# arghyasur1991/Spark-TTS

Measured on AMD Instinct MI355X. Metric: audio samples/sec (whole node), Spark-TTS-0.5B greedy, higher is better.
Workload: dtype bf16 weights + KV, fp32 activations/accumulate (LLM); vocoder: fp32 operands split into 2 bf16 planes, 3 products on the bf16 matrix pipe, fp32 accumulate

## Files before the change

### include/sparkmi_debug.h

```cpp
#ifndef SPARKMI_DEBUG_H
#define SPARKMI_DEBUG_H

#include "sparkmi.h"

#ifdef __cplusplus
extern "C" {
#endif

int smi_llm_time_kernel(smi_llm* h, int kernel, int layer, int iters, float* ms_avg, void* stream);
int smi_llm_debug_stamps(smi_llm* h, int kernel, int layer, double* out);
int smi_llm_engine(smi_llm* h, int32_t* enabled, int32_t* info, char* why, int n);
int smi_llm_set_engine(smi_llm* h, int on);
int smi_llm_engine_plan(const smi_llm_cfg* cfg, int ncu, int32_t* stats);
int smi_llm_engine_stamps(smi_llm* h, double* out, int cap);
int smi_llm_debug_hidden(smi_llm* h, float* out_host, int n);
int smi_llm_debug_read(smi_llm* h, int what, void* out_host, size_t cap, size_t* got);

int smi_llm_debug_set_kv(smi_llm* h, int layer, int slot, int pos0, int n, const float* k_host, const float* v_host);
int smi_llm_debug_get_kv(smi_llm* h, int layer, int slot, int pos0, int n, float* k_host, float* v_host);
int smi_llm_debug_layer(smi_llm* h, int layer, int M, const int32_t* rows_host, const float* hidden_host, int stage);
int smi_llm_debug_raw_stamps(smi_llm* h, unsigned long long* out, int n);
int smi_llm_debug_sample(smi_llm* h, const float* logits_host, int n_rows, uint64_t seed, int use_bound, int32_t* tokens_out);
int smi_llm_debug_penalize(smi_llm* h, const float* logits_host, int n_rows, const uint16_t* hist_host, const smi_penalty_params* pens,
                           const int32_t* emitted_host, float* logits_out, int32_t* argmax_out);
int smi_llm_debug_logprob(smi_llm* h, const float* logits_host, int n_rows, const float* temperature_host, const int32_t* tokens_host,
                          float* lp_out);

#ifdef __cplusplus
}
#endif
#endif
```

### spark-tts_amd/csrc/smi_llm.hip

```cpp
#include "smi_common.h"
#include <stdio.h>
#include <string.h>
#include <cmath>
#include <map>
#include <mutex>
#include <vector>

namespace {

constexpr int kMaxRows = SMI_MAX_ROWS;
constexpr int kHeadDim = 64;

struct RowDesc {
  int32_t slot, pos, token, flags;
};

struct SampRec {
  int32_t mode;
  int32_t top_k;
  float inv_temp, top_p;
  unsigned long long seed;
  int32_t has_seed, pad;
};

// ... 1462 lines not shown
              pk.x = smi_f32_to_bf16(s.x) | (smi_f32_to_bf16(s.y) << 16);
              pk.y = smi_f32_to_bf16(s.z) | (smi_f32_to_bf16(s.w) << 16);
              *(uint2*)((uint16_t*)base + off) = pk;
            }
          }
        }
      }
    }
  }
}

__device__ __forceinline__ int lm_tile(const int* tlist, int idx) {
  const int c = tlist[0];
  idx = idx < c ? idx : c - 1;
  return tlist[1 + (idx > 0 ? idx : 0)];
}
__device__ __forceinline__ void lm_mask4(const Ctl* ctl, int slot, int n, float4& s) {
  const AllowRec* a = &ctl->allow[slot];
  if (!allow_has(a, n + 0)) s.x = -INFINITY;
  if (!allow_has(a, n + 1)) s.y = -INFINITY;
  if (!allow_has(a, n + 2)) s.z = -INFINITY;
  if (!allow_has(a, n + 3)) s.w = -INFINITY;
}
template <int HV, int RT = 0>
__global__ __launch_bounds__(256 * HV) void k_lm(GemmP p, int ngroups_arg, int m0_launch) {
  constexpr int NTB = 2, NW = 4, U = 8, MT = 1;
  constexpr size_t kHalfBytes = (size_t)NW * NTB * MT * 1024 + 32 * 4 + NTB * 32 * 8;
  extern __shared__ __attribute__((aligned(16))) unsigned char smem_all[];
  const int half = HV == 2 ? (int)threadIdx.x >> 8 : 0;
  unsigned char* smem = smem_all + half * kHalfBytes;
  const int tid = threadIdx.x & 255, lane = tid & 63, wave = tid >> 6;
  const int KT = p.KT, NT = p.NT;
  const int m0 = m0_launch + 16 * half;
  const int M = p.M - m0 < 16 ? (p.M - m0 > 0 ? p.M - m0 : 0) : 16;
  const int ntl = RT ? p.tlist[0] : 0;
  const int ngroups = RT ? (ntl + NTB - 1) / NTB : ngroups_arg;
  float4* red = (float4*)smem;
  float* rarr = (float*)(smem + (size_t)NW * NTB * MT * 1024);
  float* bestv = rarr + 32;
  int* besti = (int*)(bestv + NTB * 32);
  const int k8 = lane >> 4, em = lane & 15;
  const int mrow = em < M ? em : (M > 0 ? M - 1 : 0);
  const int xrow = m0 + mrow < p.M ? m0 + mrow : p.M - 1;
  bf16x8 bf[U][3];
#pragma unroll
  for (int u = 0; u < U; ++u) {
// ... 7 lines not shown
#pragma unroll
    for (int u = 0; u < U; ++u) {
      int j = wave + u * NW;
      j = j < KT ? j : KT - 1;
#pragma unroll
      for (int nb = 0; nb < NTB; ++nb) {
        int nt = g * NTB + nb;
        nt = RT ? lm_tile(p.tlist, nt) : (nt < NT ? nt : NT - 1);
        w[u][nb] = smi_ldw(&p.W[((size_t)nt * KT + j) * 64 + lane]);
      }
    }
  };
  int g = blockIdx.x;
  if (g < ngroups) load_w(g);
  for (int m = wave; m < M; m += NW) {
    float v = smi_ss_lane_sum(p.sspart + (size_t)(m0 + m) * p.npart, p.npart, lane);
    v = smi_wave_sum(v);
    if (lane == 0) rarr[m] = 1.0f / sqrtf(v / (float)(KT * 32) + p.eps);
  }
  for (int i = tid; i < NTB * 32; i += 256) { bestv[i] = -INFINITY; besti[i] = 0x7fffffff; }
  __syncthreads();
  const float rn = rarr[mrow];
  for (; g < ngroups; g += gridDim.x) {
    f32x4 acc[3][NTB];
#pragma unroll
    for (int c = 0; c < 3; ++c)
#pragma unroll
      for (int a = 0; a < NTB; ++a) acc[c][a] = (f32x4){0.f, 0.f, 0.f, 0.f};
#pragma unroll
    for (int u = 0; u < U; ++u) {
      if (wave + u * NW < KT) {
#pragma unroll
        for (int nb = 0; nb < NTB; ++nb) {
          const bf16x8 a = __builtin_bit_cast(bf16x8, w[u][nb]);
          acc[2][nb] = __builtin_amdgcn_mfma_f32_16x16x32_bf16(a, bf[u][2], acc[2][nb], 0, 0, 0);
          acc[1][nb] = __builtin_amdgcn_mfma_f32_16x16x32_bf16(a, bf[u][1], acc[1][nb], 0, 0, 0);
          acc[0][nb] = __builtin_amdgcn_mfma_f32_16x16x32_bf16(a, bf[u][0], acc[0][nb], 0, 0, 0);
        }
      }
    }
    const int gn = g + gridDim.x;
    if (gn < ngroups) load_w(gn);
#pragma unroll
    for (int nb = 0; nb < NTB; ++nb) {
      const f32x4 t = (acc[2][nb] + acc[1][nb]) + acc[0][nb];
      red[(wave * NTB + nb) * 64 + lane] = make_float4(t[0], t[1], t[2], t[3]);
    }
    __syncthreads();
    if (wave < NTB) {
      const int nb = wave, nt = RT ? (g * NTB + nb < ntl ? p.tlist[1 + g * NTB + nb] : NT) : g * NTB + nb;
      if (nt < NT) {
        float4 s = red[(0 * NTB + nb) * 64 + lane];
#pragma unroll
        for (int wv = 1; wv < NW; ++wv) {
          const float4 t = red[(wv * NTB + nb) * 64 + lane];
          s.x += t.x; s.y += t.y; s.z += t.z; s.w += t.w;
        }
        s.x *= rn; s.y *= rn; s.z *= rn; s.w *= rn;
        const int n = nt * 16 + 4 * (lane >> 4);
        const bool valid = em < M;
        if (RT && valid) lm_mask4(p.ctl, p.rows[m0 + em].slot, n, s);
        if (valid && p.Y) {
          float* y = p.Y + (size_t)(m0 + em) * p.V + n;
          if (n + 0 < p.V) y[0] = s.x;
          if (n + 1 < p.V) y[1] = s.y;
          if (n + 2 < p.V) y[2] = s.z;
          if (n + 3 < p.V) y[3] = s.w;
        }
        float bv = -INFINITY;
        int bi = 0x7fffffff;
        const float sv[4] = {s.x, s.y, s.z, s.w};
#pragma unroll
        for (int r = 0; r < 4; ++r)
          if (n + r < p.V && sv[r] > bv) { bv = sv[r]; bi = n + r; }
#pragma unroll
        for (int o = 16; o <= 32; o <<= 1) {
          const float ov = __shfl_xor(bv, o, 64);
          const int oi = __shfl_xor(bi, o, 64);
          if (ov > bv || (ov == bv && oi < bi)) { bv = ov; bi = oi; }
        }
        if (lane < 16 && valid) {
          const float cv = bestv[nb * 32 + em];
          const int ci = besti[nb * 32 + em];
          if (bv > cv || (bv == cv && bi < ci)) { bestv[nb * 32 + em] = bv; besti[nb * 32 + em] = bi; }
        }
      }
    }
    __syncthreads();
  }
  if (tid < M) {
    float bv = -INFINITY;
    int bi = 0x7fffffff;
#pragma unroll
    for (int nb = 0; nb < NTB; ++nb) {
      const float ov = bestv[nb * 32 + tid];
      const int oi = besti[nb * 32 + tid];
      if (ov > bv || (ov == bv && oi < bi)) { bv = ov; bi = oi; }
    }
    p.pval[(size_t)(m0 + tid) * gridDim.x + blockIdx.x] = bv;
    p.pidx[(size_t)(m0 + tid) * gridDim.x + blockIdx.x] = bi;
  }
}


template <int UW, int RT = 0>
__global__ __launch_bounds__(256) void k_lm32(GemmP p, int ngroups_arg, int m0) {
  constexpr int NTB = 2, NW = 4, U = UW;
  extern __shared__ __attribute__((aligned(16))) unsigned char smem[];
  const int tid = threadIdx.x, lane = tid & 63, wave = tid >> 6;
  const int KT = p.KT, NT = p.NT;
  const int ntl = RT ? p.tlist[0] : 0;
  const int ngroups = RT ? (ntl + NTB - 1) / NTB : ngroups_arg;
  const int M = p.M - m0 < 32 ? p.M - m0 : 32;
  float4* red = (float4*)smem;
  float* rarr = (float*)(smem + (size_t)NW * NTB * 2 * 1024);
  float* bestv = rarr + 32;
  int* besti = (int*)(bestv + NTB * 32);
  uint4* xl = (uint4*)(smem + (size_t)NW * NTB * 2 * 1024 + 32 * 4 + NTB * 32 * 8);
  const int k8 = lane >> 4, em = lane & 15;
  const int row0 = m0 + (em < M ? em : M - 1);
  constexpr int RPW = 8;
  float ssv[RPW][4];
  const bool ss_early = p.npart <= 256;
// ... 1522 lines not shown
  uint16_t* phist;
  int32_t* pen_idx; size_t pen_idx_cap;
  std::vector<int32_t> host_pen_idx;
  float* logits; int* tok;
  float* cand_v; int* cand_i; unsigned int* cand_n;
  unsigned long long* stamps; int stamps_on;
  int max_steps;
  int tune[4];
  int graph_steps;
  int pf_inline;
  int pf_qkv_eighths;
  int prefetch_mask, prefetch_rows;
  int tune2;
  int pgemm_min_rows;
  int pg_min[4];
  int wd_parts;
  int exact;
  int gu1_lo;
  int gu1_rows;
  hipGraphExec_t graph; int graph_B, graph_seg, graph_ident, graph_samp, graph_pen, graph_lp, graph_allow;
  std::map<hipGraphExec_t, hipStream_t> graph_last;
  std::map<uint64_t, hipGraphExec_t> graph_cache;
  hipEvent_t ev0, ev1;
  std::vector<RowDesc> host_rows;
#ifdef SMI_DIAG
  EngState eng;
  int eng_on;
#endif
};

namespace {

std::vector<const void*>& lds_big_kernels() {
  static std::vector<const void*> v;
  return v;
}
bool lds_big_register(const void* f) {
  lds_big_kernels().push_back(f);
  return true;
}
template <auto F>
struct LdsBig {
  static inline const bool reg = lds_big_register((const void*)F);
};
constexpr int kLdsBigBytes = 160 * 1024;

// ... 46 lines not shown
}
bool pen_any(const smi_llm* L) {
  for (int sl = 0; sl < kMaxRows; ++sl)
    if (L->slot_pen[sl]) return true;
  return false;
}
bool lp_any(const smi_llm* L) {
  for (int sl = 0; sl < kMaxRows; ++sl)
    if (L->slot_lp[sl]) return true;
  return false;
}
bool allow_any(const smi_llm* L) {
  for (int sl = 0; sl < kMaxRows; ++sl)
    if (L->slot_allow[sl]) return true;
  return false;
}
bool lm_restricted(const smi_llm* L) {
  return L->lm_restrict && L->KTh <= 32 && !L->exact && allow_any(L);
}
bool logits_needed(const smi_llm* L) {
  return samp_any(L) || pen_any(L) || lp_any(L) || (allow_any(L) && !lm_restricted(L));
}
int allow_bits(const smi_llm* L) { return allow_any(L) ? (lm_restricted(L) ? 3 : 1) : 0; }
uint64_t graph_key(const smi_llm* L, int samp, int pen, int lp, int K) {
  return (uint64_t)L->B | ((uint64_t)L->attn_seg << 8) | ((uint64_t)(L->identity_slots ? 1 : 0) << 24) | ((uint64_t)samp << 25) |
         ((uint64_t)pen << 26) | ((uint64_t)lp << 27) | ((uint64_t)allow_bits(L) << 28) | ((uint64_t)K << 32);
}
void graphs_flush(smi_llm* L) {
  std::vector<hipStream_t> drained;
  for (auto& gl : L->graph_last) {
    bool seen = false;
    for (hipStream_t d : drained) seen |= d == gl.second;
    if (!seen) { (void)hipStreamSynchronize(gl.second); drained.push_back(gl.second); }
  }
  L->graph_last.clear();
  for (auto& kv : L->graph_cache) if (kv.second) (void)hipGraphExecDestroy(kv.second);
  L->graph_cache.clear();
  L->graph = nullptr;
}

template <int MT, int NTB, int NW, int U, int WB, int PRO, int EPI, int H = 1, int OCC = 1>
int launch_gemm_kv(const smi_llm* L, GemmP p, hipStream_t st) {
  const int work = (p.NT + NTB - 1) / NTB * H;
  p.work_blocks = work;
  p.stamps = L->stamps_on ? L->stamps : nullptr;
  if constexpr (MT == 1 && NTB == 1 && NW == 16 && H == 4 && PRO == PRO_PLAIN && EPI == EPI_RESID) {
    if (p.M == 1 && !p.stamps && p.KT <= 160 && !(L->tune2 & 1048576)) {
      const int helpers = (L->prefetch_mask & 4) && p.pf.base && work < 232 ? ((L->tune2 & 4194304) ? 224 : (256 - work) / 8 * 8) : 0;
      if (p.KT <= 32) hipLaunchKernelGGL(k_down1<2>, dim3(work + helpers), dim3(256), 0, st, p);
// ... 458 lines not shown
      p.XSout = L->xs_h; p.ssout = L->sspart;
      p.gamma_next = layer + 1 < c.num_layers ? (const float*)sec(L, SMI_LLM_LN1, layer + 1)
                                              : (const float*)sec(L, SMI_LLM_FINAL_NORM, 0);
      if (layer + 1 < c.num_layers) p.pf = PfDesc{sec(L, SMI_LLM_WQKV, layer + 1), L->KTh * 1024, L->NTqkv, 0, (L->NTqkv + 7) / 8};
      if (M >= L->dc_min && M <= kMaxRows && !L->tune[3] && !L->stamps_on && p.KT <= 160 && p.NT % 4 == 0)
        return launch_down_chains(L, p, st);
      switch (L->tune[3]) {
        case 2: return launch_gemm<1, 16, 3, 4, PRO_PLAIN, EPI_RESID>(L, p, st);
        case 4: return launch_gemm<1, 8, 10, 2, PRO_PLAIN, EPI_RESID>(L, p, st);
        case 5: return launch_gemm<1, 16, 2, 5, PRO_PLAIN, EPI_RESID, 2>(L, p, st);
        case 6: return launch_gemm<1, 16, 2, 5, PRO_PLAIN, EPI_RESID>(L, p, st);
        default:
          if (M <= 8) return launch_gemm<1, 16, 2, 5, PRO_PLAIN, EPI_RESID, 4>(L, p, st);
          if (M <= 16) return launch_gemm<1, 16, 2, 5, PRO_PLAIN, EPI_RESID, 4, 0>(L, p, st);
          if (M <= 32) return launch_gemm<1, 16, 2, 5, PRO_PLAIN, EPI_RESID, 2, 0>(L, p, st);
          return launch_gemm<1, 16, 2, 5, PRO_PLAIN, EPI_RESID, 1, 0>(L, p, st);
      }
    case KLM:
      p.W = (const uint4*)sec(L, SMI_LLM_LM_HEAD, 0); p.NT = L->NTlm; p.KT = L->KTh;
      p.XS = L->xs_h;
      p.Y = logits ? logits : (logits_needed(L) ? L->logits : nullptr);
      p.V = c.vocab_size; p.pval = L->pval; p.pidx = L->pidx;
      p.stamps = L->stamps_on ? L->stamps : nullptr;
      if (L->KTh <= 32 && !logits && rows == L->rows && lm_restricted(L)) {
        p.tlist = L->tlist; p.ctl = L->ctl;
        const size_t lds = (size_t)4 * 2 * 1024 + 32 * 4 + 2 * 32 * 8;
        const size_t lds32 = (size_t)4 * 2 * 2 * 1024 + 32 * 4 + 2 * 32 * 8 + (size_t)L->KTh * 12 * 16 * 16;
        if (M <= 16) {
          hipLaunchKernelGGL((k_lm<1, 1>), dim3(L->lm_blocks), dim3(256), lds, st, p, 0, 0);
          SMI_LAUNCH_CHECK();
          return SMI_OK;
        }
        for (int m0 = 0; m0 < M; m0 += 32) {
          if (!(L->tune2 & 8192) && lds32 <= 150 * 1024) {
            if (L->KTh <= 28) hipLaunchKernelGGL((k_lm32<7, 1>), dim3(lm_blocks_for(L, M)), dim3(256), lds32, st, p, 0, m0);
            else hipLaunchKernelGGL((k_lm32<8, 1>), dim3(lm_blocks_for(L, M)), dim3(256), lds32, st, p, 0, m0);
          } else
            hipLaunchKernelGGL((k_lm<2, 1>), dim3(lm_blocks_for(L, M)), dim3(512), 2 * lds, st, p, 0, m0);
          SMI_LAUNCH_CHECK();
        }
        return SMI_OK;
      }
      if (L->KTh <= 32) {
        const int ngroups = (L->NTlm + 1) / 2;
        const size_t lds = (size_t)4 * 2 * 1024 + 32 * 4 + 2 * 32 * 8;
        if (M <= 16) {
// ... 408 lines not shown
  {
    static std::mutex mu;
    static bool done[64] = {};
    int dev = 0;
    std::lock_guard<std::mutex> lk(mu);
    if (hipGetDevice(&dev) != hipSuccess || dev < 0 || dev >= 64) {
      smi_set_error("smi_llm_create: no current device");
      smi_llm_destroy(L);
      return SMI_EHIP;
    }
    for (size_t i = 0; i < lds_big_kernels().size() && !done[dev]; ++i)
      if (hipFuncSetAttribute(lds_big_kernels()[i], hipFuncAttributeMaxDynamicSharedMemorySize, kLdsBigBytes) != hipSuccess) {
        smi_set_error("smi_llm_create: hipFuncSetAttribute(MaxDynamicSharedMemorySize) failed: %s", hipGetErrorString(hipGetLastError()));
        smi_llm_destroy(L);
        return SMI_EHIP;
      }
    done[dev] = true;
  }
  if (hipEventCreate(&L->ev0) != hipSuccess || hipEventCreate(&L->ev1) != hipSuccess) {
    smi_set_error("hipEventCreate failed");
    smi_llm_destroy(L);
    return SMI_EHIP;
  }
#ifdef SMI_DIAG
  L->eng_on = 0;
  snprintf(L->eng.why, sizeof(L->eng.why), "off (opt-in: SPARKMI_ENGINE=1 or smi_llm_set_engine)");
  { const char* e = smi_env("SPARKMI_ENGINE");
    if (e && e[0] == '1') {
      const int rce = eng_create(L);
      if (rce) { smi_llm_destroy(L); return rce; }
      L->eng_on = L->eng.enabled;
    }
  }
#endif
  *out = L;
  return SMI_OK;
}

int smi_llm_destroy(smi_llm* L) {
  if (!L) return SMI_OK;
  graphs_flush(L);
  eng_destroy(L);
  void* ptrs[] = {L->h, L->qbuf, L->xs_h, L->xs_attn, L->xs_act, L->sspart, L->part_o, L->h2, L->dpart, L->fuse_cnt, L->rows, L->plan, L->pf_tiles, L->pval, L->pidx, L->hist,
                  L->count, L->finished, L->step, L->ctl, L->ptab, L->kcache, L->vcache, L->logits, L->tok, L->cand_v, L->cand_i, L->cand_n, L->stamps, L->bh, L->bq, L->bxs_h, L->bxs_attn, L->bxs_act, L->bss, L->pslab, L->apart,
                  L->phist, L->pen_idx, L->lp, L->lp_part, L->lp_rowc, L->tlist};
  for (void* q : ptrs)
    if (q) (void)hipFree(q);
  if (L->ev0) (void)hipEventDestroy(L->ev0);
  if (L->ev1) (void)hipEventDestroy(L->ev1);
  delete L;
  return SMI_OK;
}

int smi_llm_set_sampling(smi_llm* L, int do_sample, float temperature, int top_k, float top_p, uint64_t seed) {
  SMI_REQUIRE(L, "smi_llm_set_sampling: null handle");
  if (do_sample) {
    SMI_REQUIRE(temperature > 0.f, "smi_llm_set_sampling: temperature must be > 0");
    SMI_REQUIRE(top_k >= 1 && top_k <= kSampleCap, "smi_llm_set_sampling: top_k must be in 1..%d", kSampleCap);
    SMI_REQUIRE(top_p > 0.f && top_p <= 1.f, "smi_llm_set_sampling: top_p must be in (0, 1]");
    if (top_k > L->cfg.vocab_size) top_k = L->cfg.vocab_size;
  }
  const bool changed = L->do_sample != (do_sample ? 1 : 0) ||
                       (do_sample && (L->temperature != temperature || L->top_k != top_k || L->top_p != top_p));
  L->do_sample = do_sample ? 1 : 0;
  L->temperature = temperature; L->top_k = top_k; L->top_p = top_p; L->seed = seed;
  L->hctl.seed = seed;
  SMI_HIP(hipMemcpy(&L->ctl->seed, &seed, sizeof(seed), hipMemcpyHostToDevice));
  if (changed) graphs_flush(L);
// ... 965 lines not shown

int smi_llm_engine(smi_llm* L, int32_t* enabled, int32_t* info, char* why, int n) {
  SMI_REQUIRE(L, "smi_llm_engine: null handle");
  if (enabled) *enabled = L->eng.enabled && L->eng_on;
  if (info) { info[0] = L->eng.ncu; info[1] = L->eng.maxlen; info[2] = L->eng.lds; info[3] = L->eng.enabled; }
  if (why && n > 0) { strncpy(why, L->eng.why, (size_t)n - 1); why[n - 1] = 0; }
  return SMI_OK;
}

int smi_llm_set_engine(smi_llm* L, int on) {
  SMI_REQUIRE(L, "smi_llm_set_engine: null handle");
  int v = on ? 1 : 0;
  if (v && !L->eng.enabled) {
    SMI_HIP(hipDeviceSynchronize());
    const int rce = eng_create(L);
    if (rce) return rce;
    v = L->eng.enabled;
  }
  if (v != L->eng_on) { SMI_HIP(hipDeviceSynchronize()); graphs_flush(L); }
  L->eng_on = v;
  return SMI_OK;
}

int smi_llm_engine_plan(const smi_llm_cfg* cfg, int ncu, int32_t* stats) {
  SMI_REQUIRE(cfg_ok(cfg) && stats, "smi_llm_engine_plan: invalid argument");
  EngPlanHost P;
  char why[128] = "";
  const int Q = cfg->num_heads * cfg->head_dim, KV = cfg->num_kv_heads * cfg->head_dim;
  if (!eng_build_plan(cfg->hidden_size, Q, KV, cfg->intermediate_size, cfg->num_heads, ncu, P, why, sizeof(why))) {
    smi_set_error("engine plan: %s", why);
    return SMI_EINVAL;
  }
  long total = 0, want = 0;
  for (int ph = 0; ph < 4; ++ph) want += (long)P.g.nparts[ph] * P.g.part_imgs[ph];
  std::vector<unsigned char> seen[4];
  for (int ph = 0; ph < 4; ++ph) seen[ph].assign((size_t)P.g.nparts[ph] * 4 * 64, 0);
  for (int c = 0; c < ncu; ++c)
    for (int w = 0; w < kEngWaves; ++w) {
      const EngWavePlan& wp = P.cu[c].w[w];
      for (int ph = 0; ph < 4; ++ph)
        for (int j = wp.jstart[ph]; j < wp.jstart[ph + 1]; ++j) {
          const EngJob& jb = wp.jobs[j];
          SMI_REQUIRE(P.cu[c].parts[P.cu[c].pstart[ph] + jb.slot] == jb.part, "engine plan: job slot does not name its part");
          SMI_REQUIRE((int)jb.goff + jb.nimg <= (int)P.cu[c].len_cu, "engine plan: job beyond the CU's stream");
          for (int r = 0; r < jb.nimg; ++r) {
            const uint32_t d = P.desc[(size_t)c * P.maxlen + jb.goff + r];
// ... 14 lines not shown

int smi_llm_debug_hidden(smi_llm* L, float* out_host, int n) {
  SMI_REQUIRE(L && out_host && n >= L->H, "smi_llm_debug_hidden: out holds %d floats, %d needed", n, L ? L->H : 0);
  SMI_HIP(hipDeviceSynchronize());
  SMI_HIP(hipMemcpy(out_host, L->h, (size_t)L->H * 4, hipMemcpyDeviceToHost));
  return eng_check(L);
}

int smi_llm_debug_read(smi_llm* L, int what, void* out_host, size_t cap, size_t* got) {
  SMI_REQUIRE(L && out_host && got, "smi_llm_debug_read: null argument");
  const void* src = nullptr;
  size_t n = 0;
  const size_t R = L->B > 0 ? (size_t)L->B : 1;
  switch (what) {
    case 0: src = L->qbuf; n = R * L->Q * 4; break;
    case 1: src = L->xs_attn; n = R * L->Q * 6; break;
    case 2: src = L->xs_act; n = R * L->I * 6; break;
    case 3: src = L->xs_h; n = R * L->H * 6; break;
    case 4: src = L->h; n = R * L->H * 4; break;
    case 5: src = L->eng.gran; n = L->eng.gran ? (size_t)2 * L->eng.gran_per_buf * 8 : 0; break;
    case 6: src = L->sspart; n = R * L->H; break;
    case 7: src = L->kcache; n = (size_t)L->cfg.max_positions * kHeadDim * 2; break;
    case 8: src = L->h2; n = (size_t)L->H * 4; break;
    default: smi_set_error("smi_llm_debug_read: what=%d", what); return SMI_EINVAL;
  }
  SMI_REQUIRE(src && n <= cap, "smi_llm_debug_read: buffer %d holds %zu bytes, out holds %zu", what, n, cap);
  SMI_HIP(hipDeviceSynchronize());
  SMI_HIP(hipMemcpy(out_host, src, n, hipMemcpyDeviceToHost));
  *got = n;
  return SMI_OK;
}

static int debug_kv_check(const smi_llm* L, int layer, int slot, int pos0, int n) {
  SMI_REQUIRE(L && !L->paged, "debug KV access needs a contiguous KV cache (kv_page_tokens = 0)");
  SMI_REQUIRE(layer >= 0 && layer < L->cfg.num_layers && slot >= 0 && slot < L->cfg.max_slots && pos0 >= 0 && n >= 0 &&
              pos0 + n <= L->cfg.max_positions, "debug KV access: layer %d slot %d positions %d..%d out of range", layer, slot, pos0, pos0 + n);
  return SMI_OK;
}

int smi_llm_debug_set_kv(smi_llm* L, int layer, int slot, int pos0, int n, const float* k_host, const float* v_host) {
  { const int rc = debug_kv_check(L, layer, slot, pos0, n); if (rc) return rc; }
  SMI_REQUIRE(k_host && v_host, "smi_llm_debug_set_kv: null argument");
  SMI_HIP(hipDeviceSynchronize());
  const int nkv = L->cfg.num_kv_heads, f32 = L->cfg.kv_dtype;
  const size_t esz = f32 ? 4 : 2;
  std::vector<unsigned char> buf((size_t)n * kHeadDim * esz);
// ... 256 lines not shown
```

### spark-tts_amd/sparkmi/_lib.py

```python
from __future__ import annotations

import ctypes as C
import os
from pathlib import Path

_HERE = Path(__file__).resolve().parent
LIB_PATH = Path(os.environ["SPARKMI_LIB"]) if os.environ.get("SPARKMI_LIB") else _HERE / "libsparkmi.so"

SMI_MAX_ROWS = 64
SMI_MAX_EOS = 4
ABI_VERSION = 4


class SparkMIError(RuntimeError):
    pass


class LLMCfg(C.Structure):
    _fields_ = [(n, C.c_int32) for n in (
        "vocab_size", "hidden_size", "num_layers", "num_heads", "num_kv_heads", "head_dim",
        "intermediate_size", "max_slots", "max_positions", "kv_dtype", "use_graph")] + [("rms_eps", C.c_float),
                                                                                        ("kv_page_tokens", C.c_int32), ("kv_pages", C.c_int32), ("wd_plain", C.c_int32),
                                                                                        ("weights_exact", C.c_int32)]

# ... 100 lines not shown
    "smi_voc_num_launches": (_I, [_VP]),
    "smi_voc_time_launch": (_I, [_VP, _I, _I, _P(C.c_float), _P(C.c_double), C.c_char_p, _I, _VP]),
    "smi_voc_block_arena_count": (_I, [_P(VocBlockCfg)]),
    "smi_voc_block_arena_bytes": (_SZ, [_P(VocBlockCfg)]),
    "smi_voc_block_arena_entry": (_I, [_P(VocBlockCfg), _I, C.c_char_p, _I, _P(_SZ), _P(_SZ), _P(C.c_int32)]),
    "smi_voc_block_run": (_I, [_P(VocBlockCfg), _VP, _SZ, _VP, _VP, _VP, _P(C.c_int32), _I, _I, _VP, _VP]),
    "smi_enc_arena_count": (_I, [_P(EncCfg)]),
    "smi_enc_arena_entry": (_I, [_P(EncCfg), _I, C.c_char_p, _I, _P(_SZ), _P(_SZ), _P(C.c_int32)]),
    "smi_enc_arena_bytes": (_SZ, [_P(EncCfg)]),
    "smi_enc_create": (_I, [_P(EncCfg), _VP, _SZ, _P(_VP)]),
    "smi_enc_destroy": (_I, [_VP]),
    "smi_enc_forward": (_I, [_VP, _VP, _I, _VP, _I, _VP, _VP, _P(_I), _VP]),
    "smi_enc_debug_stage": (_I, [_VP, C.c_char_p, _VP, _SZ, _P(C.c_int32), _VP]),
    "smi_enc_num_launches": (_I, [_VP]),
    "smi_enc_time_launch": (_I, [_VP, _I, _I, _P(C.c_float), _P(C.c_double), C.c_char_p, _I, _VP]),
}

DEBUG_SYMBOLS = {
    "smi_llm_time_kernel": (_I, [_VP, _I, _I, _I, _P(C.c_float), _VP]),
    "smi_llm_debug_stamps": (_I, [_VP, _I, _I, _P(C.c_double)]),
    "smi_llm_engine": (_I, [_VP, _P(C.c_int32), _P(C.c_int32), C.c_char_p, _I]),
    "smi_llm_set_engine": (_I, [_VP, _I]),
    "smi_llm_engine_plan": (_I, [_P(LLMCfg), _I, _P(C.c_int32)]),
    "smi_llm_engine_stamps": (_I, [_VP, _P(C.c_double), _I]),
    "smi_llm_debug_hidden": (_I, [_VP, _P(C.c_float), _I]),
    "smi_llm_debug_read": (_I, [_VP, _I, _VP, _SZ, _P(_SZ)]),
    "smi_llm_debug_raw_stamps": (_I, [_VP, _P(C.c_uint64), _I]),
    "smi_llm_debug_sample": (_I, [_VP, _P(C.c_float), _I, C.c_uint64, _I, _P(C.c_int32)]),
    "smi_llm_debug_logprob": (_I, [_VP, _P(C.c_float), _I, _P(C.c_float), _P(C.c_int32), _P(C.c_float)]),
    "smi_llm_debug_penalize": (_I, [_VP, _P(C.c_float), _I, _P(C.c_uint16), _P(PenaltyParams), _P(C.c_int32), _P(C.c_float),
                                    _P(C.c_int32)]),
    "smi_llm_debug_set_kv": (_I, [_VP, _I, _I, _I, _I, _P(C.c_float), _P(C.c_float)]),
    "smi_llm_debug_get_kv": (_I, [_VP, _I, _I, _I, _I, _P(C.c_float), _P(C.c_float)]),
    "smi_llm_debug_layer": (_I, [_VP, _I, _I, _P(C.c_int32), _P(C.c_float), _I]),
}

DIAG_PATH = LIB_PATH.with_name("libsparkmi_diag.so")


class _Lib:

    def __init__(self, cdll: C.CDLL, path: Path, is_diag: bool):
        self._cdll, self.path, self.is_diag = cdll, path, is_diag

    def __getattr__(self, name):
        return getattr(self._cdll, name)
# ... 56 lines not shown
```

### spark-tts_amd/sparkmi/llm.py

```python
from __future__ import annotations

import ctypes as C
import itertools
import json
import warnings
from pathlib import Path
from typing import Iterable, List, Mapping, Optional, Sequence, Union

import numpy as np
import torch

from . import _lib
from .arena import llm_cfg_struct, pack_llm_arena
from .config import LLMConfig


EosLike = Union[None, int, Iterable[int]]
SAMPLING_KEYS = ("do_sample", "temperature", "top_k", "top_p", "seed")
PENALTY_KEYS = ("repetition_penalty", "presence_penalty", "frequency_penalty", "min_new_tokens", "penalize_prompt")
PENALTY_NEUTRAL = dict(repetition_penalty=1.0, presence_penalty=0.0, frequency_penalty=0.0, min_new_tokens=0)
LOGPROB_KEYS = ("return_log_probs",)
ALLOW_KEY = "allowed_token_ids"


# ... 585 lines not shown
        self._lib.check(self._lib.smi_llm_forward_logits(
            self._h, a.ctypes.data_as(C.POINTER(C.c_int64)), a.shape[0], C.c_void_p(out.data_ptr()),
            self._stream()), "smi_llm_forward_logits")
        return out

    def _need_diag(self, what: str) -> None:
        if not self._lib.is_diag:
            raise _lib.SparkMIError(f"SparkLLM.{what} is a diagnostics entry (include/sparkmi_debug.h): construct the engine with "
                                    "diag=True (libsparkmi_diag.so); the product library does not export it")

    def engine_info(self) -> dict:
        self._need_diag("engine_info")
        on = C.c_int32(0)
        info = (C.c_int32 * 4)()
        why = C.create_string_buffer(200)
        self._lib.check(self._lib.smi_llm_engine(self._h, C.byref(on), info, why, 200), "smi_llm_engine")
        return {"enabled": bool(on.value), "built": bool(info[3]), "cus": int(info[0]), "images_per_wave": int(info[1]),
                "lds_bytes": int(info[2]), "why": why.value.decode(errors="replace")}

    def set_engine(self, on: bool) -> None:
        self._need_diag("set_engine")
        self._lib.check(self._lib.smi_llm_set_engine(self._h, 1 if on else 0), "smi_llm_set_engine")

    def engine_stamps(self) -> np.ndarray:
        self._need_diag("engine_stamps")
        n = 3 * self.cfg.num_hidden_layers * 16
        out = (C.c_double * n)()
        self._lib.check(self._lib.smi_llm_engine_stamps(self._h, out, n), "smi_llm_engine_stamps")
        return np.array(out, dtype=np.float64).reshape(3, self.cfg.num_hidden_layers, 16)

    def debug_hidden(self) -> np.ndarray:
        self._need_diag("debug_hidden")
        out = np.zeros(self.cfg.hidden_size, dtype=np.float32)
        self._lib.check(self._lib.smi_llm_debug_hidden(self._h, out.ctypes.data_as(C.POINTER(C.c_float)), out.size), "smi_llm_debug_hidden")
        return out

    def debug_read(self, what: int) -> np.ndarray:
        self._need_diag("debug_read")
        buf = np.zeros(1 << 22, dtype=np.uint8)
        got = C.c_size_t(0)
        self._lib.check(self._lib.smi_llm_debug_read(self._h, int(what), buf.ctypes.data_as(C.c_void_p), buf.size, C.byref(got)),
                   "smi_llm_debug_read")
        return buf[: got.value].copy()

    def debug_set_kv(self, layer: int, slot: int, k: np.ndarray, v: np.ndarray, pos0: int = 0) -> None:
        self._need_diag("debug_set_kv")
# ... 126 lines not shown
```

Before: 564,600.

## Screen lm_head argmax with int8 bounds and recompute only candidate tiles exactly

Adds an int8 copy of the lm_head with per-row scales and error bounds, built once at create. For single-row greedy decode it runs an int8 MFMA screen that computes interval bounds on each logit, finds the max lower bound, then recomputes the exact bf16 3-plane GEMM only for vocab tiles whose upper bound can reach it. This is meant to cut the memory traffic and MFMA work of the full-vocab lm_head GEMV per token. It adds two kernel launches, extra device memory and bound-soundness risk; argmax stays exact when the bounds are correct.

```diff
diff --git a/include/sparkmi_debug.h b/include/sparkmi_debug.h
--- a/include/sparkmi_debug.h
+++ b/include/sparkmi_debug.h
@@ -13,6 +13,7 @@
 int smi_llm_set_engine(smi_llm* h, int on);
 int smi_llm_engine_plan(const smi_llm_cfg* cfg, int ncu, int32_t* stats);
 int smi_llm_engine_stamps(smi_llm* h, double* out, int cap);
+int smi_llm_debug_lm_screen(smi_llm* h, int mode, int64_t* info);
 int smi_llm_debug_hidden(smi_llm* h, float* out_host, int n);
 int smi_llm_debug_read(smi_llm* h, int what, void* out_host, size_t cap, size_t* got);
 
diff --git a/spark-tts_amd/csrc/smi_llm.hip b/spark-tts_amd/csrc/smi_llm.hip
--- a/spark-tts_amd/csrc/smi_llm.hip
+++ b/spark-tts_amd/csrc/smi_llm.hip
@@ -1508,6 +1508,53 @@
   if (!allow_has(a, n + 2)) s.z = -INFINITY;
   if (!allow_has(a, n + 3)) s.w = -INFINITY;
 }
+template <int U, int NTB, int NW>
+__device__ __forceinline__ void lm_group_acc(const uint4 (&w)[U][NTB], const bf16x8 (&bf)[U][3], int wave, int KT, f32x4 (&t)[NTB]) {
+  f32x4 acc[3][NTB];
+#pragma unroll
+  for (int c = 0; c < 3; ++c)
+#pragma unroll
+    for (int a = 0; a < NTB; ++a) acc[c][a] = (f32x4){0.f, 0.f, 0.f, 0.f};
+#pragma unroll
+  for (int u = 0; u < U; ++u) {
+    if (wave + u * NW < KT) {
+#pragma unroll
+      for (int nb = 0; nb < NTB; ++nb) {
+        const bf16x8 a = __builtin_bit_cast(bf16x8, w[u][nb]);
+        acc[2][nb] = __builtin_amdgcn_mfma_f32_16x16x32_bf16(a, bf[u][2], acc[2][nb], 0, 0, 0);
+        acc[1][nb] = __builtin_amdgcn_mfma_f32_16x16x32_bf16(a, bf[u][1], acc[1][nb], 0, 0, 0);
+        acc[0][nb] = __builtin_amdgcn_mfma_f32_16x16x32_bf16(a, bf[u][0], acc[0][nb], 0, 0, 0);
+      }
+    }
+  }
+#pragma unroll
+  for (int nb = 0; nb < NTB; ++nb) t[nb] = (acc[2][nb] + acc[1][nb]) + acc[0][nb];
+}
+template <int NTB, int NW>
+__device__ __forceinline__ float4 lm_group_sum(const float4* red, int nb, int lane, float rn) {
+  float4 s = red[(0 * NTB + nb) * 64 + lane];
+#pragma unroll
+  for (int wv = 1; wv < NW; ++wv) {
+    const float4 t = red[(wv * NTB + nb) * 64 + lane];
+    s.x += t.x; s.y += t.y; s.z += t.z; s.w += t.w;
+  }
+  s.x *= rn; s.y *= rn; s.z *= rn; s.w *= rn;
+  return s;
+}
+__device__ __forceinline__ void lm_tile_best(const float4& s, int n, int V, float& bv, int& bi) {
+  bv = -INFINITY;
+  bi = 0x7fffffff;
+  const float sv[4] = {s.x, s.y, s.z, s.w};
+#pragma unroll
+  for (int r = 0; r < 4; ++r)
+    if (n + r < V && sv[r] > bv) { bv = sv[r]; bi = n + r; }
+#pragma unroll
+  for (int o = 16; o <= 32; o <<= 1) {
+    const float ov = __shfl_xor(bv, o, 64);
+    const int oi = __shfl_xor(bi, o, 64);
+    if (ov > bv || (ov == bv && oi < bi)) { bv = ov; bi = oi; }
+  }
+}
 template <int HV, int RT = 0>
 __global__ __launch_bounds__(256 * HV) void k_lm(GemmP p, int ngroups_arg, int m0_launch) {
   constexpr int NTB = 2, NW = 4, U = 8, MT = 1;
@@ -1561,41 +1608,17 @@
   __syncthreads();
   const float rn = rarr[mrow];
   for (; g < ngroups; g += gridDim.x) {
-    f32x4 acc[3][NTB];
-#pragma unroll
-    for (int c = 0; c < 3; ++c)
-#pragma unroll
-      for (int a = 0; a < NTB; ++a) acc[c][a] = (f32x4){0.f, 0.f, 0.f, 0.f};
-#pragma unroll
-    for (int u = 0; u < U; ++u) {
-      if (wave + u * NW < KT) {
-#pragma unroll
-        for (int nb = 0; nb < NTB; ++nb) {
-          const bf16x8 a = __builtin_bit_cast(bf16x8, w[u][nb]);
-          acc[2][nb] = __builtin_amdgcn_mfma_f32_16x16x32_bf16(a, bf[u][2], acc[2][nb], 0, 0, 0);
-          acc[1][nb] = __builtin_amdgcn_mfma_f32_16x16x32_bf16(a, bf[u][1], acc[1][nb], 0, 0, 0);
-          acc[0][nb] = __builtin_amdgcn_mfma_f32_16x16x32_bf16(a, bf[u][0], acc[0][nb], 0, 0, 0);
-        }
-      }
-    }
+    f32x4 t[NTB];
+    lm_group_acc<U, NTB, NW>(w, bf, wave, KT, t);
     const int gn = g + gridDim.x;
     if (gn < ngroups) load_w(gn);
 #pragma unroll
-    for (int nb = 0; nb < NTB; ++nb) {
-      const f32x4 t = (acc[2][nb] + acc[1][nb]) + acc[0][nb];
-      red[(wave * NTB + nb) * 64 + lane] = make_float4(t[0], t[1], t[2], t[3]);
-    }
+    for (int nb = 0; nb < NTB; ++nb) red[(wave * NTB + nb) * 64 + lane] = make_float4(t[nb][0], t[nb][1], t[nb][2], t[nb][3]);
     __syncthreads();
     if (wave < NTB) {
       const int nb = wave, nt = RT ? (g * NTB + nb < ntl ? p.tlist[1 + g * NTB + nb] : NT) : g * NTB + nb;
       if (nt < NT) {
-        float4 s = red[(0 * NTB + nb) * 64 + lane];
-#pragma unroll
-        for (int wv = 1; wv < NW; ++wv) {
-          const float4 t = red[(wv * NTB + nb) * 64 + lane];
-          s.x += t.x; s.y += t.y; s.z += t.z; s.w += t.w;
-        }
-        s.x *= rn; s.y *= rn; s.z *= rn; s.w *= rn;
+        float4 s = lm_group_sum<NTB, NW>(red, nb, lane, rn);
         const int n = nt * 16 + 4 * (lane >> 4);
         const bool valid = em < M;
         if (RT && valid) lm_mask4(p.ctl, p.rows[m0 + em].slot, n, s);
@@ -1606,18 +1629,9 @@
           if (n + 2 < p.V) y[2] = s.z;
           if (n + 3 < p.V) y[3] = s.w;
         }
-        float bv = -INFINITY;
-        int bi = 0x7fffffff;
-        const float sv[4] = {s.x, s.y, s.z, s.w};
-#pragma unroll
-        for (int r = 0; r < 4; ++r)
-          if (n + r < p.V && sv[r] > bv) { bv = sv[r]; bi = n + r; }
-#pragma unroll
-        for (int o = 16; o <= 32; o <<= 1) {
-          const float ov = __shfl_xor(bv, o, 64);
-          const int oi = __shfl_xor(bi, o, 64);
-          if (ov > bv || (ov == bv && oi < bi)) { bv = ov; bi = oi; }
-        }
+        float bv;
+        int bi;
+        lm_tile_best(s, n, p.V, bv, bi);
         if (lane < 16 && valid) {
           const float cv = bestv[nb * 32 + em];
           const int ci = besti[nb * 32 + em];
@@ -1638,6 +1652,260 @@
     }
     p.pval[(size_t)(m0 + tid) * gridDim.x + blockIdx.x] = bv;
     p.pidx[(size_t)(m0 + tid) * gridDim.x + blockIdx.x] = bi;
+  }
+}
+
+constexpr int kLmqU = 14;
+struct LmqP {
+  const uint4* Q;
+  const float4* meta;
+  const unsigned char* XS;
+  const float* sspart; int npart; float eps;
+  int KT, NT, V, nper;
+  float* hi;
+  float* wmax;
+};
+
+__global__ __launch_bounds__(256) void k_lmq_build(const uint16_t* W, int KT, int8_t* Q, float4* meta) {
+  __shared__ float smx[16][17];
+  __shared__ double sd[16][17];
+  const int tid = threadIdx.x, r = tid & 15, part = tid >> 4, nt = blockIdx.x, K = KT * 32, KJ = KT / 2;
+  auto wv = [&](int k) {
+    const size_t tile = (size_t)nt * KT + (k >> 5);
+    return smi_bf16_to_f32(W[tile * 512 + (((k >> 3) & 3) * 16 + r) * 8 + (k & 7)]);
+  };
+  float mx = 0.f;
+  double l1 = 0.0;
+  bool nan = false;
+  for (int k = part; k < K; k += 16) { const float w = fabsf(wv(k)); nan |= !(w == w); mx = fmaxf(mx, w); l1 += (double)w; }
+  smx[part][r] = nan ? INFINITY : mx; sd[part][r] = l1;
+  __syncthreads();
+  mx = 0.f; l1 = 0.0;
+  for (int i = 0; i < 16; ++i) { mx = fmaxf(mx, smx[i][r]); l1 += sd[i][r]; }
+  __syncthreads();
+  const bool ok = mx > 0.f && mx < INFINITY;
+  const float s = ok ? mx / 127.0f : 0.f, inv = ok ? 127.0f / mx : 0.f;
+  double e = 0.0;
+  for (int k = part; k < K; k += 16) {
+    const float w = wv(k);
+    float q = rintf(w * inv);
+    q = fminf(fmaxf(q, -127.f), 127.f);
+    if (!(q == q)) q = 0.f;
+    e = fmax(e, fabs((double)w - (double)s * (double)q));
+    Q[(((size_t)nt * KJ + (k >> 6)) * 64 + ((k >> 4) & 3) * 16 + r) * 16 + (k & 15)] = (int8_t)(int)q;
+  }
+  sd[part][r] = e;
+  __syncthreads();
+  if (part == 0) {
+    e = 0.0;
+    for (int i = 0; i < 16; ++i) e = fmax(e, sd[i][r]);
+    float ef = __double2float_ru(e), lf = __double2float_ru(l1);
+    if (!(mx < INFINITY)) { ef = INFINITY; lf = INFINITY; }
+    meta[(size_t)nt * 16 + r] = make_float4(s, ef, lf, 0.f);
+  }
+}
+
+__global__ __launch_bounds__(256) __attribute__((amdgpu_waves_per_eu(4, 4))) void k_lm_screen(LmqP p) {
+  typedef int i32x4 __attribute__((ext_vector_type(4)));
+  __shared__ __attribute__((aligned(16))) int8_t xh_s[kLmqU * 64];
+  __shared__ __attribute__((aligned(16))) int8_t xl_s[kLmqU * 64];
+  __shared__ float redf[4];
+  __shared__ double redd[2][4];
+  __shared__ float rn_s;
+  const int tid = threadIdx.x, lane = tid & 63, wave = tid >> 6;
+  const int KT = p.KT, KJ = KT >> 1, K = KT * 32, NT = p.NT;
+  const int gw = blockIdx.x * 4 + wave;
+  const int t0 = gw * p.nper, t1 = t0 + p.nper < NT ? t0 + p.nper : NT;
+  uint4 w[kLmqU];
+  float4 mt = make_float4(0.f, 0.f, 0.f, 0.f);
+  auto load_w = [&](int nt) {
+#pragma unroll
+    for (int j = 0; j < kLmqU; ++j) w[j] = smi_ldw(&p.Q[((size_t)nt * KJ + (j < KJ ? j : KJ - 1)) * 64 + lane]);
+    mt = p.meta[(size_t)nt * 16 + (lane & 15)];
+  };
+  if (t0 < t1) load_w(t0);
+  float x[4] = {0.f, 0.f, 0.f, 0.f};
+  const int k0 = 4 * tid;
+  if (k0 < K) {
+    const size_t o = xs_off(k0 >> 5, 0, (k0 >> 3) & 3, 0, 1) + (k0 & 7) * 2;
+    const size_t pl = (size_t)4 * 16;
+    const uint2 h = *(const uint2*)(p.XS + o), m = *(const uint2*)(p.XS + o + pl), l = *(const uint2*)(p.XS + o + 2 * pl);
+    const uint32_t hu[2] = {h.x, h.y}, mu[2] = {m.x, m.y}, lu[2] = {l.x, l.y};
+#pragma unroll
+    for (int e = 0; e < 4; ++e) {
+      const int sh = (e & 1) * 16;
+      x[e] = (smi_bf16_to_f32((hu[e >> 1] >> sh) & 0xffffu) + smi_bf16_to_f32((mu[e >> 1] >> sh) & 0xffffu)) + smi_bf16_to_f32((lu[e >> 1] >> sh) & 0xffffu);
+    }
+  }
+  if (wave == 0) {
+    float v = smi_ss_lane_sum(p.sspart, p.npart, lane);
+    v = smi_wave_sum(v);
+    if (lane == 0) rn_s = 1.0f / sqrtf(v / (float)(KT * 32) + p.eps);
+  }
+  float amax = fmaxf(fmaxf(fabsf(x[0]), fabsf(x[1])), fmaxf(fabsf(x[2]), fabsf(x[3])));
+  int bad = !(x[0] == x[0] && x[1] == x[1] && x[2] == x[2] && x[3] == x[3]);
+#pragma unroll
+  for (int o = 32; o > 0; o >>= 1) { amax = fmaxf(amax, __shfl_xor(amax, o, 64)); bad |= __shfl_xor(bad, o, 64); }
+  if (lane == 0) redf[wave] = bad ? INFINITY : amax;
+  __syncthreads();
+  amax = fmaxf(fmaxf(redf[0], redf[1]), fmaxf(redf[2], redf[3]));
+  const bool live = amax > 0.f && amax < INFINITY;
+  const float sx = live ? amax / 127.0f : 0.f, inv = live ? 127.0f / amax : 0.f;
+  double x1 = 0.0, eo = 0.0;
+  if (k0 < K) {
+    uint32_t ph = 0, pl2 = 0;
+#pragma unroll
+    for (int e = 0; e < 4; ++e) {
+      float h = rintf(x[e] * inv);
+      h = fminf(fmaxf(h, -127.f), 127.f);
+      float l = rintf((x[e] - sx * h) * inv * 127.0f);
+      l = fminf(fmaxf(l, -127.f), 127.f);
+      if (!live) { h = 0.f; l = 0.f; }
+      const double xhat = (double)sx * ((double)h + (double)l / 127.0);
+      x1 += fabs(xhat);
+      eo = fmax(eo, fabs((double)x[e] - xhat));
+      ph |= ((uint32_t)(int)h & 0xffu) << (8 * e);
+      pl2 |= ((uint32_t)(int)l & 0xffu) << (8 * e);
+    }
+    *(uint32_t*)&xh_s[k0] = ph;
+    *(uint32_t*)&xl_s[k0] = pl2;
+  }
+#pragma unroll
+  for (int o = 32; o > 0; o >>= 1) {
+    x1 += __shfl_xor(x1, o, 64);
+    eo = fmax(eo, __shfl_xor(eo, o, 64));
+  }
+  if (lane == 0) { redd[0][wave] = x1; redd[1][wave] = eo; }
+  __syncthreads();
+  x1 = ((redd[0][0] + redd[0][1]) + redd[0][2]) + redd[0][3];
+  eo = fmax(fmax(redd[1][0], redd[1][1]), fmax(redd[1][2], redd[1][3]));
+  const float rn = rn_s;
+  const float X1 = __double2float_ru(x1 * (1.0 + 1e-9));
+  const float cop = live ? __double2float_ru((eo + (double)K * (1.0 / 4194304.0) * (double)amax) * (1.0 + 1e-9)) : 0.f;
+  const bool sane = amax < INFINITY && rn == rn && rn < INFINITY;
+  const int8_t* xsrc = ((lane & 15) == 0 ? xh_s : xl_s) + (lane >> 4) * 16;
+  const bool xrow = (lane & 15) <= 1;
+  const float c127 = 1.0f / 127.0f, up = 1.0f + 0.0009765625f, aslack = 9.5367431640625e-07f;
+  float best_lo = -INFINITY;
+  for (int nt = t0; nt < t1; ++nt) {
+    i32x4 acc = {0, 0, 0, 0};
+#pragma unroll
+    for (int j = 0; j < kLmqU; ++j)
+      if (j < KJ) {
+        i32x4 xa = *(const i32x4*)&xsrc[j * 64];
+        if (!xrow) xa = (i32x4){0, 0, 0, 0};
+        acc = __builtin_amdgcn_mfma_i32_16x16x64_i8(xa, __builtin_bit_cast(i32x4, w[j]), acc, 0, 0, 0);
+      }
+    const float4 me = mt;
+    if (nt + 1 < t1) load_w(nt + 1);
+    if (lane < 16) {
+      const int id = nt * 16 + lane;
+      const float a = (rn * me.x * sx) * ((float)acc[0] + (float)acc[1] * c127);
+      const float b = rn * (me.y * X1 + me.z * cop) * up + fabsf(a) * aslack + 1e-30f;
+      float lo = a - b, hi = a + b;
+      if (!sane || !(fabsf(a) < INFINITY) || !(b < INFINITY)) { lo = -INFINITY; hi = INFINITY; }
+      if (id >= p.V) { lo = -INFINITY; hi = -INFINITY; }
+      p.hi[id] = hi;
+      best_lo = fmaxf(best_lo, lo);
+    }
+  }
+#pragma unroll
+  for (int o = 8; o > 0; o >>= 1) best_lo = fmaxf(best_lo, __shfl_xor(best_lo, o, 64));
+  if (lane == 0) p.wmax[gw] = best_lo;
+}
+
+__global__ __launch_bounds__(256) void k_lm_pick(GemmP p, const float* hi, const float* wmax, int nwmax, int per, int force, unsigned* ncand_out) {
+  constexpr int NTB = 2, NW = 4, U = 8;
+  __shared__ float4 red[NW * NTB * 64];
+  __shared__ float tmax_s[4];
+  __shared__ float rn_s;
+  __shared__ int ncand_s;
+  extern __shared__ int cand_s[];
+  const int tid = threadIdx.x, lane = tid & 63, wave = tid >> 6, k8 = lane >> 4;
+  const int KT = p.KT, NT = p.NT;
+  bf16x8 bf[U][3];
+#pragma unroll
+  for (int u = 0; u < U; ++u) {
+    int j = wave + u * NW;
+    j = j < KT ? j : KT - 1;
+#pragma unroll
+    for (int s = 0; s < 3; ++s) bf[u][s] = *(const bf16x8*)(p.XS + xs_off(j, s, k8, 0, 1));
+  }
+  float tm = -INFINITY;
+  for (int i = tid; i < nwmax; i += 256) tm = fmaxf(tm, wmax[i]);
+  if (wave == 0) {
+    float v = smi_ss_lane_sum(p.sspart, p.npart, lane);
+    v = smi_wave_sum(v);
+    if (lane == 0) rn_s = 1.0f / sqrtf(v / (float)(KT * 32) + p.eps);
+  }
+#pragma unroll
+  for (int o = 32; o > 0; o >>= 1) tm = fmaxf(tm, __shfl_xor(tm, o, 64));
+  if (lane == 0) tmax_s[wave] = tm;
+  __syncthreads();
+  const float T = force ? -INFINITY : fmaxf(fmaxf(tmax_s[0], tmax_s[1]), fmaxf(tmax_s[2], tmax_s[3]));
+  const int tb = blockIdx.x * per;
+  for (int i = tid; i < per; i += 256) {
+    const int nt = tb + i;
+    int c = 0;
+    if (nt < NT) {
+      const float4* h4 = (const float4*)(hi + (size_t)nt * 16);
+#pragma unroll
+      for (int q = 0; q < 4; ++q) { const float4 v = h4[q]; c += (v.x >= T) + (v.y >= T) + (v.z >= T) + (v.w >= T); }
+      if (force) c = 16;
+    }
+    cand_s[i] = c;
+  }
+  __syncthreads();
+  if (tid == 0) {
+    int n = 0, ids = 0;
+    for (int i = 0; i < per; ++i)
+      if (cand_s[i]) { ids += cand_s[i]; cand_s[n++] = tb + i; }
+    ncand_s = n;
+    if (ncand_out && ids) atomicAdd(ncand_out, (unsigned)ids);
+  }
+  __syncthreads();
+  const int nc = ncand_s;
+  const float rn = rn_s;
+  float bestv = -INFINITY;
+  int besti = 0x7fffffff;
+  for (int c = 0; c < nc; c += NTB) {
+    uint4 w[U][NTB];
+    int nts[NTB];
+#pragma unroll
+    for (int nb = 0; nb < NTB; ++nb) nts[nb] = cand_s[c + nb < nc ? c + nb : nc - 1];
+#pragma unroll
+    for (int u = 0; u < U; ++u) {
+      int j = wave + u * NW;
+      j = j < KT ? j : KT - 1;
+#pragma unroll
+      for (int nb = 0; nb < NTB; ++nb) w[u][nb] = smi_ldw(&p.W[((size_t)nts[nb] * KT + j) * 64 + lane]);
+    }
+    f32x4 t[NTB];
+    lm_group_acc<U, NTB, NW>(w, bf, wave, KT, t);
+#pragma unroll
+    for (int nb = 0; nb < NTB; ++nb) red[(wave * NTB + nb) * 64 + lane] = make_float4(t[nb][0], t[nb][1], t[nb][2], t[nb][3]);
+    __syncthreads();
+    if (wave < NTB) {
+      const float4 s = lm_group_sum<NTB, NW>(red, wave, lane, rn);
+      float bv;
+      int bi;
+      lm_tile_best(s, nts[wave] * 16 + 4 * (lane >> 4), p.V, bv, bi);
+      bv = __shfl(bv, 0, 64); bi = __shfl(bi, 0, 64);
+      if (bv > bestv || (bv == bestv && bi < besti)) { bestv = bv; besti = bi; }
+    }
+    __syncthreads();
+  }
+  float* rf = (float*)red;
+  if (wave < NTB && lane == 0) { rf[wave] = bestv; ((int*)rf)[8 + wave] = besti; }
+  __syncthreads();
+  if (tid == 0) {
+    float bv = rf[0];
+    int bi = ((int*)rf)[8];
+    const float ov = rf[1];
+    const int oi = ((int*)rf)[9];
+    if (ov > bv || (ov == bv && oi < bi)) { bv = ov; bi = oi; }
+    p.pval[blockIdx.x] = bv;
+    p.pidx[blockIdx.x] = bi;
   }
 }
 
@@ -3206,6 +3474,12 @@
   std::map<hipGraphExec_t, hipStream_t> graph_last;
   std::map<uint64_t, hipGraphExec_t> graph_cache;
   hipEvent_t ev0, ev1;
+  int8_t* lmq; float4* lmq_meta;
+  float* lmq_hi; float* lmq_wmax;
+  unsigned* lmq_ncand;
+  int lmq_nper, lmq_blocks;
+  int lmq_mode;
+  long long lmq_launches;
   std::vector<RowDesc> host_rows;
 #ifdef SMI_DIAG
   EngState eng;
@@ -3298,9 +3572,13 @@
   return samp_any(L) || pen_any(L) || lp_any(L) || (allow_any(L) && !lm_restricted(L));
 }
 int allow_bits(const smi_llm* L) { return allow_any(L) ? (lm_restricted(L) ? 3 : 1) : 0; }
+bool lm_screen_step(const smi_llm* L, int M) {
+  return L->lmq && L->lmq_mode && M == 1 && !L->exact && !logits_needed(L) && !allow_any(L) && !L->stamps_on;
+}
 uint64_t graph_key(const smi_llm* L, int samp, int pen, int lp, int K) {
   return (uint64_t)L->B | ((uint64_t)L->attn_seg << 8) | ((uint64_t)(L->identity_slots ? 1 : 0) << 24) | ((uint64_t)samp << 25) |
-         ((uint64_t)pen << 26) | ((uint64_t)lp << 27) | ((uint64_t)allow_bits(L) << 28) | ((uint64_t)K << 32);
+         ((uint64_t)pen << 26) | ((uint64_t)lp << 27) | ((uint64_t)allow_bits(L) << 28) |
+         ((uint64_t)(lm_screen_step(L, L->B) ? 1 : 0) << 30) | ((uint64_t)K << 32);
 }
 void graphs_flush(smi_llm* L) {
   std::vector<hipStream_t> drained;
@@ -3805,6 +4083,23 @@
       p.Y = logits ? logits : (logits_needed(L) ? L->logits : nullptr);
       p.V = c.vocab_size; p.pval = L->pval; p.pidx = L->pidx;
       p.stamps = L->stamps_on ? L->stamps : nullptr;
+      if (!logits && rows == L->rows && lm_screen_step(L, M) && !eng_usable(L, rows, M)) {
+        LmqP q;
+        q.Q = (const uint4*)L->lmq; q.meta = L->lmq_meta; q.XS = L->xs_h; q.sspart = L->sspart; q.npart = p.npart; q.eps = p.eps;
+        q.KT = L->KTh; q.NT = L->NTlm; q.V = c.vocab_size; q.nper = L->lmq_nper; q.hi = L->lmq_hi; q.wmax = L->lmq_wmax;
+        hipLaunchKernelGGL(k_lm_screen, dim3(L->lmq_blocks), dim3(256), 0, st, q);
+        SMI_LAUNCH_CHECK();
+        const int per = (L->NTlm + L->lm_blocks - 1) / L->lm_blocks;
+        unsigned* ncand = nullptr;
+#ifdef SMI_DIAG
+        ncand = L->lmq_ncand;
+#endif
+        hipLaunchKernelGGL(k_lm_pick, dim3(L->lm_blocks), dim3(256), (size_t)per * 4, st, p, (const float*)L->lmq_hi, (const float*)L->lmq_wmax,
+                           L->lmq_blocks * 4, per, L->lmq_mode == 2 ? 1 : 0, ncand);
+        SMI_LAUNCH_CHECK();
+        ++L->lmq_launches;
+        return SMI_OK;
+      }
       if (L->KTh <= 32 && !logits && rows == L->rows && lm_restricted(L)) {
         p.tlist = L->tlist; p.ctl = L->ctl;
         const size_t lds = (size_t)4 * 2 * 1024 + 32 * 4 + 2 * 32 * 8;
@@ -4259,6 +4554,30 @@
     smi_llm_destroy(L);
     return SMI_EHIP;
   }
+  L->lmq_mode = 1;
+  if (const char* e = smi_env("SPARKMI_LM_SCREEN")) L->lmq_mode = atoi(e) == 0 ? 0 : atoi(e) == 2 ? 2 : 1;
+  if (!L->exact && L->KTh % 2 == 0 && L->KTh / 2 <= kLmqU) {
+    const size_t nid = (size_t)L->NTlm * 16;
+    const int nper = L->NTlm / 2048 > 0 ? L->NTlm / 2048 : 1;
+    const int waves = (L->NTlm + nper - 1) / nper;
+    L->lmq_nper = nper; L->lmq_blocks = (waves + 3) / 4;
+    if (hipMalloc((void**)&L->lmq, nid * (size_t)L->H) != hipSuccess || hipMalloc((void**)&L->lmq_meta, nid * sizeof(float4)) != hipSuccess ||
+        hipMalloc((void**)&L->lmq_hi, nid * 4) != hipSuccess || hipMalloc((void**)&L->lmq_wmax, (size_t)L->lmq_blocks * 4 * 4) != hipSuccess ||
+        hipMalloc((void**)&L->lmq_ncand, 4) != hipSuccess || hipMemset(L->lmq_ncand, 0, 4) != hipSuccess) {
+      (void)hipGetLastError();
+      void* q4[] = {L->lmq, L->lmq_meta, L->lmq_hi, L->lmq_wmax, L->lmq_ncand};
+      for (void* q : q4)
+        if (q) (void)hipFree(q);
+      L->lmq = nullptr; L->lmq_meta = nullptr; L->lmq_hi = nullptr; L->lmq_wmax = nullptr; L->lmq_ncand = nullptr;
+    } else {
+      hipLaunchKernelGGL(k_lmq_build, dim3(L->NTlm), dim3(256), 0, 0, (const uint16_t*)sec(L, SMI_LLM_LM_HEAD, 0), L->KTh, L->lmq, L->lmq_meta);
+      if (hipGetLastError() != hipSuccess || hipDeviceSynchronize() != hipSuccess) {
+        smi_set_error("smi_llm_create: building the lm_head screen's int8 copy failed");
+        smi_llm_destroy(L);
+        return SMI_EHIP;
+      }
+    }
+  }
 #ifdef SMI_DIAG
   L->eng_on = 0;
   snprintf(L->eng.why, sizeof(L->eng.why), "off (opt-in: SPARKMI_ENGINE=1 or smi_llm_set_engine)");
@@ -4280,7 +4599,7 @@
   eng_destroy(L);
   void* ptrs[] = {L->h, L->qbuf, L->xs_h, L->xs_attn, L->xs_act, L->sspart, L->part_o, L->h2, L->dpart, L->fuse_cnt, L->rows, L->plan, L->pf_tiles, L->pval, L->pidx, L->hist,
                   L->count, L->finished, L->step, L->ctl, L->ptab, L->kcache, L->vcache, L->logits, L->tok, L->cand_v, L->cand_i, L->cand_n, L->stamps, L->bh, L->bq, L->bxs_h, L->bxs_attn, L->bxs_act, L->bss, L->pslab, L->apart,
-                  L->phist, L->pen_idx, L->lp, L->lp_part, L->lp_rowc, L->tlist};
+                  L->phist, L->pen_idx, L->lp, L->lp_part, L->lp_rowc, L->tlist, L->lmq, L->lmq_meta, L->lmq_hi, L->lmq_wmax, L->lmq_ncand};
   for (void* q : ptrs)
     if (q) (void)hipFree(q);
   if (L->ev0) (void)hipEventDestroy(L->ev0);
@@ -5292,6 +5611,21 @@
   return SMI_OK;
 }
 
+int smi_llm_debug_lm_screen(smi_llm* L, int mode, int64_t* info) {
+  SMI_REQUIRE(L && mode >= -1 && mode <= 2, "smi_llm_debug_lm_screen: bad argument");
+  SMI_HIP(hipDeviceSynchronize());
+  if (mode >= 0 && mode != L->lmq_mode) { graphs_flush(L); L->lmq_mode = mode; }
+  if (info) {
+    unsigned nc = 0;
+    if (L->lmq_ncand) {
+      SMI_HIP(hipMemcpy(&nc, L->lmq_ncand, 4, hipMemcpyDeviceToHost));
+      SMI_HIP(hipMemset(L->lmq_ncand, 0, 4));
+    }
+    info[0] = L->lmq ? 1 : 0; info[1] = L->lmq_mode; info[2] = L->lmq_launches; info[3] = nc;
+  }
+  return SMI_OK;
+}
+
 int smi_llm_engine_plan(const smi_llm_cfg* cfg, int ncu, int32_t* stats) {
   SMI_REQUIRE(cfg_ok(cfg) && stats, "smi_llm_engine_plan: invalid argument");
   EngPlanHost P;
@@ -5352,6 +5686,8 @@
     case 6: src = L->sspart; n = R * L->H; break;
     case 7: src = L->kcache; n = (size_t)L->cfg.max_positions * kHeadDim * 2; break;
     case 8: src = L->h2; n = (size_t)L->H * 4; break;
+    case 9: src = L->pval; n = R * (size_t)lm_blocks_for(L, (int)R) * 4; break;
+    case 10: src = L->pidx; n = R * (size_t)lm_blocks_for(L, (int)R) * 4; break;
     default: smi_set_error("smi_llm_debug_read: what=%d", what); return SMI_EINVAL;
   }
   SMI_REQUIRE(src && n <= cap, "smi_llm_debug_read: buffer %d holds %zu bytes, out holds %zu", what, n, cap);
diff --git a/spark-tts_amd/sparkmi/_lib.py b/spark-tts_amd/sparkmi/_lib.py
--- a/spark-tts_amd/sparkmi/_lib.py
+++ b/spark-tts_amd/sparkmi/_lib.py
@@ -146,6 +146,7 @@
     "smi_llm_engine": (_I, [_VP, _P(C.c_int32), _P(C.c_int32), C.c_char_p, _I]),
     "smi_llm_set_engine": (_I, [_VP, _I]),
     "smi_llm_engine_plan": (_I, [_P(LLMCfg), _I, _P(C.c_int32)]),
+    "smi_llm_debug_lm_screen": (_I, [_VP, _I, _P(C.c_int64)]),
     "smi_llm_engine_stamps": (_I, [_VP, _P(C.c_double), _I]),
     "smi_llm_debug_hidden": (_I, [_VP, _P(C.c_float), _I]),
     "smi_llm_debug_read": (_I, [_VP, _I, _VP, _SZ, _P(_SZ)]),
diff --git a/spark-tts_amd/sparkmi/llm.py b/spark-tts_amd/sparkmi/llm.py
--- a/spark-tts_amd/sparkmi/llm.py
+++ b/spark-tts_amd/sparkmi/llm.py
@@ -631,6 +631,12 @@
         self._need_diag("set_engine")
         self._lib.check(self._lib.smi_llm_set_engine(self._h, 1 if on else 0), "smi_llm_set_engine")
 
+    def lm_screen(self, mode: Optional[int] = None) -> dict:
+        self._need_diag("lm_screen")
+        info = (C.c_int64 * 4)()
+        self._lib.check(self._lib.smi_llm_debug_lm_screen(self._h, -1 if mode is None else int(mode), info), "smi_llm_debug_lm_screen")
+        return {"built": bool(info[0]), "mode": int(info[1]), "launches": int(info[2]), "candidates": int(info[3])}
+
     def engine_stamps(self) -> np.ndarray:
         self._need_diag("engine_stamps")
         n = 3 * self.cfg.num_hidden_layers * 16
```

New measurement: 570,400, median of 6. 1.01x the previous value.
